# LayerXcom/zero-chain

Measured on NVIDIA H100. Metric: g1_msm_mops_2^20, higher is better.
Workload: dtype u32-limb Montgomery (Fq 12x32, Fr 8x32), integer

## Files before the change

zero_chain_b200/csrc/curve.cuh:

```cuda
#pragma once
#include "field.cuh"

struct Fq2 {
    Fq c0, c1;
    ZK_DEV static Fq2 zero() { Fq2 r; r.c0 = Fq::zero(); r.c1 = Fq::zero(); return r; }
    ZK_DEV static Fq2 one() { Fq2 r; r.c0 = Fq::one(); r.c1 = Fq::zero(); return r; }
    ZK_DEV bool is_zero() const { return c0.is_zero() && c1.is_zero(); }
    ZK_DEV bool operator==(const Fq2 &b) const { return c0 == b.c0 && c1 == b.c1; }
    ZK_DEV bool operator!=(const Fq2 &b) const { return !(*this == b); }
    ZK_DEV friend Fq2 operator+(const Fq2 &a, const Fq2 &b) { Fq2 r; r.c0 = a.c0 + b.c0; r.c1 = a.c1 + b.c1; return r; }
    ZK_DEV friend Fq2 operator-(const Fq2 &a, const Fq2 &b) { Fq2 r; r.c0 = a.c0 - b.c0; r.c1 = a.c1 - b.c1; return r; }
    ZK_DEV Fq2 dbl() const { Fq2 r; r.c0 = c0.dbl(); r.c1 = c1.dbl(); return r; }
    ZK_DEV Fq2 neg() const { Fq2 r; r.c0 = c0.neg(); r.c1 = c1.neg(); return r; }
    ZK_DEV Fq2 cneg(bool f) const { return f ? neg() : *this; }
    ZK_F2FN friend Fq2 operator*(const Fq2 &a, const Fq2 &b) {
        Fq aa = a.c0 * b.c0, bb = a.c1 * b.c1;
        Fq t = (a.c0 + a.c1) * (b.c0 + b.c1);
        Fq2 r; r.c1 = t - aa - bb; r.c0 = aa - bb; return r;
    }
    ZK_F2FN Fq2 sqr() const {
        Fq ab = c0 * c1;
        Fq2 r; r.c0 = (c0 + c1) * (c0 - c1); r.c1 = ab.dbl(); return r;
    }
    ZK_DEV Fq2 inverse() const {
        Fq n = (c0.sqr() + c1.sqr()).inverse();
        Fq2 r; r.c0 = c0 * n; r.c1 = (c1 * n).neg(); return r;
    }
};

template <class F>
struct Affine {
    F x, y;
    ZK_DEV bool is_inf() const { return x.is_zero() && y.is_zero(); }
    ZK_DEV static Affine inf() { Affine r; r.x = F::zero(); r.y = F::zero(); return r; }
};

template <class F>
struct XYZZ {
    F x, y, zz, zzz;
    ZK_DEV static XYZZ inf() { XYZZ r; r.x = F::zero(); r.y = F::zero(); r.zz = F::zero(); r.zzz = F::zero(); return r; }
    ZK_DEV bool is_inf() const { return zz.is_zero(); }
    ZK_DEV static XYZZ from_affine(const Affine<F> &p) {
        XYZZ r;
        if (p.is_inf()) return inf();
        r.x = p.x; r.y = p.y; r.zz = F::one(); r.zzz = F::one(); return r;
    }
    ZK_DEV XYZZ neg() const { XYZZ r = *this; r.y = y.neg(); return r; }

    ZK_PTFN static XYZZ dbl_affine(const Affine<F> &p) {
        if (p.is_inf()) return inf();
        F u = p.y.dbl(), v = u.sqr(), w = u * v, s = p.x * v;
        F xx = p.x.sqr(), m = xx.dbl() + xx;
        XYZZ r;
        r.x = m.sqr() - s.dbl();
        r.y = m * (s - r.x) - w * p.y;
        r.zz = v; r.zzz = w;
        return r;
    }
    ZK_PTFN XYZZ dbl() const {
        if (is_inf()) return *this;
        F u = y.dbl(), v = u.sqr(), w = u * v, s = x * v;
        F xx = x.sqr(), m = xx.dbl() + xx;
        XYZZ r;
        r.x = m.sqr() - s.dbl();
        r.y = m * (s - r.x) - w * y;
        r.zz = v * zz; r.zzz = w * zzz;
        return r;
    }
    ZK_PTFN void add_mixed(const Affine<F> &p) {
        if (p.is_inf()) return;
        if (is_inf()) { x = p.x; y = p.y; zz = F::one(); zzz = F::one(); return; }
        F u2 = p.x * zz, s2 = p.y * zzz;
        F pp_ = u2 - x, r = s2 - y;
        if (pp_.is_zero()) {
            if (r.is_zero()) *this = dbl_affine(p); else *this = inf();
            return;
        }
        F pp = pp_.sqr(), ppp = pp_ * pp, q = x * pp;
        F x3 = r.sqr() - ppp - q.dbl();
        y = r * (q - x3) - y * ppp;
        x = x3;
        zz = zz * pp; zzz = zzz * ppp;
    }
    ZK_PTFN void add(const XYZZ &o) {
        if (o.is_inf()) return;
        if (is_inf()) { *this = o; return; }
        F u1 = x * o.zz, u2 = o.x * zz, s1 = y * o.zzz, s2 = o.y * zzz;
        F pp_ = u2 - u1, r = s2 - s1;
        if (pp_.is_zero()) {
            if (r.is_zero()) *this = dbl(); else *this = inf();
            return;
        }
        F pp = pp_.sqr(), ppp = pp_ * pp, q = u1 * pp;
        F x3 = r.sqr() - ppp - q.dbl();
        y = r * (q - x3) - s1 * ppp;
        x = x3;
        zz = zz * o.zz * pp; zzz = zzz * o.zzz * ppp;
    }
    ZK_PTFN Affine<F> to_affine() const {
        if (is_inf()) return Affine<F>::inf();
        F zi = zzz.inverse();
        F zi2 = (zi * zz).sqr();
        Affine<F> r; r.x = x * zi2; r.y = y * zi; return r;
    }
};

template <class F>
ZK_PTFN XYZZ<F> scalar_mul(const XYZZ<F> &p, const uint32_t *k) {
    XYZZ<F> acc = XYZZ<F>::inf();
    bool started = false;
    for (int i = 255; i >= 0; i--) {
        if (started) acc = acc.dbl();
        if ((k[i >> 5] >> (i & 31)) & 1) { acc.add(p); started = true; }
    }
    return acc;
}

typedef Affine<Fq> G1Affine;
typedef Affine<Fq2> G2Affine;
typedef XYZZ<Fq> G1XYZZ;
typedef XYZZ<Fq2> G2XYZZ;
```

zero_chain_b200/csrc/curve_coop.cuh:

```cuda
#pragma once
#include "curve.cuh"

namespace zkcoop {

template <class F>
__device__ __forceinline__ F bcast(const F &v, int src) {
    F r;
    const uint32_t *s = reinterpret_cast<const uint32_t *>(&v);
    uint32_t *d = reinterpret_cast<uint32_t *>(&r);
#pragma unroll
    for (int k = 0; k < (int)(sizeof(F) / 4); k++) d[k] = __shfl_sync(0xffffffffu, s[k], src);
    return r;
}
template <class F>
__device__ __forceinline__ F pick(int lane, const F &c0, const F &c1, const F &c2, const F &c3) {
    F r;
    const uint32_t *p0 = reinterpret_cast<const uint32_t *>(&c0), *p1 = reinterpret_cast<const uint32_t *>(&c1);
    const uint32_t *p2 = reinterpret_cast<const uint32_t *>(&c2), *p3 = reinterpret_cast<const uint32_t *>(&c3);
    uint32_t *d = reinterpret_cast<uint32_t *>(&r);
#pragma unroll
    for (int k = 0; k < (int)(sizeof(F) / 4); k++) d[k] = lane == 1 ? p1[k] : (lane == 2 ? p2[k] : (lane == 3 ? p3[k] : p0[k]));
    return r;
}

template <class F>
__device__ __noinline__ void dbl(XYZZ<F> &P) {
    if (P.is_inf()) return;
    const int lane = threadIdx.x & 31;
    const F U = P.y.dbl();
    F a = pick(lane, U, P.x, U, U), p = a * a;
    const F V = bcast(p, 0), XX = bcast(p, 1);
    const F M = XX.dbl() + XX;
    a = pick(lane, U, P.x, M, U);
    F b = pick(lane, V, V, M, V);
    p = a * b;
    const F W = bcast(p, 0), S = bcast(p, 1), MM = bcast(p, 2);
    const F X3 = MM - S.dbl();
    a = pick(lane, M, W, V, W);
    b = pick(lane, S - X3, P.y, P.zz, P.zzz);
    p = a * b;
    const F t0 = bcast(p, 0), t1 = bcast(p, 1);
    P.zz = bcast(p, 2); P.zzz = bcast(p, 3);
    P.x = X3; P.y = t0 - t1;
}

template <class F>
__device__ __noinline__ void add(XYZZ<F> &P, const XYZZ<F> &Q) {
    if (Q.is_inf()) return;
    if (P.is_inf()) { P = Q; return; }
    const int lane = threadIdx.x & 31;
    F a = pick(lane, P.x, Q.x, P.y, Q.y), b = pick(lane, Q.zz, P.zz, Q.zzz, P.zzz), p = a * b;
    const F U1 = bcast(p, 0), U2 = bcast(p, 1), S1 = bcast(p, 2), S2 = bcast(p, 3);
    const F Pd = U2 - U1, R = S2 - S1;
    if (Pd.is_zero()) {
        if (R.is_zero()) dbl(P); else P = XYZZ<F>::inf();
        return;
    }
    a = pick(lane, Pd, R, P.zz, P.zzz); b = pick(lane, Pd, R, Q.zz, Q.zzz); p = a * b;
    const F PP = bcast(p, 0), RR = bcast(p, 1), ZZ12 = bcast(p, 2), ZZZ12 = bcast(p, 3);
    a = pick(lane, Pd, U1, ZZ12, Pd); p = a * PP;
    const F PPP = bcast(p, 0), Qv = bcast(p, 1);
    P.zz = bcast(p, 2);
    const F X3 = RR - PPP - Qv.dbl();
    a = pick(lane, R, S1, ZZZ12, R); b = pick(lane, Qv - X3, PPP, PPP, PPP); p = a * b;
    const F t0 = bcast(p, 0), t1 = bcast(p, 1);
    P.zzz = bcast(p, 2);
    P.x = X3; P.y = t0 - t1;
}

}
```

zero_chain_b200/csrc/engine.cu:

```cuda
#define ZK_SEMI_HOT 1
#include "internal.h"
#include "msm_driver.cuh"

using namespace zkmsm;

static thread_local char g_err[512] = "";
void zk_set_error(const char *fmt, ...) {
    va_list ap; va_start(ap, fmt); vsnprintf(g_err, sizeof(g_err), fmt, ap); va_end(ap);
    (void)cudaGetLastError();
}
extern "C" const char *zk_last_error(void) { return g_err; }
extern "C" const char *zk_version(void) { return "zkb200 0.1 (sm_90a)"; }
extern "C" int zk_device_count(void) {
    int n = 0;
    if (cudaGetDeviceCount(&n) != cudaSuccess) { cudaGetLastError(); return 0; }
    return n;
}
int zk_use_device(zk_ctx *ctx) { ZK_CUDA(cudaSetDevice(ctx->device)); return ZK_OK; }

extern "C" int zk_ctx_create(int device, void *stream, zk_ctx **out) {
    if (!out) { zk_set_error("zk_ctx_create: out is NULL"); return ZK_ERR_INVALID; }
    int n = zk_device_count();
    if (n == 0) { zk_set_error("no CUDA device: libzkb200 has no CPU fallback"); return ZK_ERR_CUDA; }
    if (device < 0 || device >= n) { zk_set_error("device %d out of range (%d devices)", device, n); return ZK_ERR_INVALID; }
// ... 244 lines not shown
    ctx->pending_bytes = 0;
    ZK_CUDA(cudaEventSynchronize(ctx->ev_tail));
    ZK_TRY(zk_check_err_flag(ctx));
    memcpy(out, ctx->h_pinned, per);
    return ZK_OK;
}
extern "C" size_t zk_partial_size(int group) { return group == 1 ? sizeof(G1XYZZ) : sizeof(G2XYZZ); }
extern "C" int zk_msm_partial_device(zk_ctx *ctx, const zk_bases *b, const void *d_scalars, size_t n, void *d_partial_out) {
    if (!d_partial_out) { zk_set_error("zk_msm_partial_device: out is NULL"); return ZK_ERR_INVALID; }
    ZK_TRY(zk_msm_run(ctx, b, d_scalars, n, 1));
    ZK_CUDA(cudaMemcpyAsync(d_partial_out, ctx->result.p, zk_partial_size(b->group), cudaMemcpyDeviceToDevice, ctx->stream));
    return zk_check_err_flag(ctx);
}
extern "C" int zk_points_fold(zk_ctx *ctx, int group, const void *d_partials, size_t count, uint8_t *out) {
    if (!ctx || !d_partials || !out || count == 0) { zk_set_error("zk_points_fold: bad argument"); return ZK_ERR_INVALID; }
    ZK_TRY(zk_use_device(ctx));
    ZK_TRY(ctx->result.reserve(4 * sizeof(G2XYZZ)));
    if (group == 1) k_fold_serial<Fq><<<1, 32, 0, ctx->stream>>>((const G1XYZZ *)d_partials, (int)count, ctx->result.as<G1XYZZ>());
    else k_fold_serial<Fq2><<<1, 32, 0, ctx->stream>>>((const G2XYZZ *)d_partials, (int)count, ctx->result.as<G2XYZZ>());
    ZK_CUDA(cudaGetLastError());
    return zk_encode_results(ctx, group, 1, 0, out);
}

template <class F>
__global__ void __launch_bounds__(128) k_scalar_mul_many(const Affine<F> *base, const uint32_t *scalars, size_t n, Affine<F> *out) {
    size_t i = (size_t)blockIdx.x * blockDim.x + threadIdx.x;
    if (i >= n) return;
    uint32_t k[8];
    for (int j = 0; j < 8; j++) k[j] = scalars[i * 8 + j];
    out[i] = scalar_mul(XYZZ<F>::from_affine(base[0]), k).to_affine();
}
extern "C" int zk_scalar_mul_many(zk_ctx *ctx, int group, const uint64_t *base, const uint64_t *scalars, size_t n, uint64_t *out) {
    if (!ctx || !base || !scalars || !out) { zk_set_error("zk_scalar_mul_many: NULL argument"); return ZK_ERR_INVALID; }
    if (group != 1 && group != 2) { zk_set_error("group must be 1 or 2"); return ZK_ERR_INVALID; }
    ZK_TRY(zk_use_device(ctx));
    size_t psz = group == 1 ? sizeof(G1Affine) : sizeof(G2Affine);
    ZK_TRY(ctx->stage_a.reserve(psz)); ZK_TRY(ctx->stage_b.reserve(n * 32)); ZK_TRY(ctx->stage_c.reserve(n * psz));
    ZK_CUDA(cudaMemcpyAsync(ctx->stage_a.p, base, psz, cudaMemcpyHostToDevice, ctx->stream));
    ZK_CUDA(cudaMemcpyAsync(ctx->stage_b.p, scalars, n * 32, cudaMemcpyHostToDevice, ctx->stream));
    unsigned blk = (unsigned)((n + 127) / 128);
    if (group == 1) k_scalar_mul_many<Fq><<<blk, 128, 0, ctx->stream>>>(ctx->stage_a.as<G1Affine>(), ctx->stage_b.as<uint32_t>(), n, ctx->stage_c.as<G1Affine>());
    else k_scalar_mul_many<Fq2><<<blk, 128, 0, ctx->stream>>>(ctx->stage_a.as<G2Affine>(), ctx->stage_b.as<uint32_t>(), n, ctx->stage_c.as<G2Affine>());
    ZK_CUDA(cudaGetLastError());
    ZK_CUDA(cudaMemcpyAsync(out, ctx->stage_c.p, n * psz, cudaMemcpyDeviceToHost, ctx->stream));
    ZK_CUDA(cudaStreamSynchronize(ctx->stream));
    return ZK_OK;
}

template <class T>
__global__ void k_field_op(int op, const T *a, const T *b, size_t n, T *out) {
    size_t i = (size_t)blockIdx.x * blockDim.x + threadIdx.x;
    if (i >= n) return;
    T x = a[i], y = b ? b[i] : x, r;
    switch (op) {
    case 0: r = x * y; break;
    case 1: r = x + y; break;
    case 2: r = x - y; break;
    case 3: r = x.sqr(); break;
    case 4: r = x.inverse(); break;
    case 5: r = T::canonical_lt_mod(x) ? T::from_canonical(x) : T::zero(); break;
    default: r = x.to_canonical(); break;
    }
    out[i] = r;
}
extern "C" int zk_field_op(zk_ctx *ctx, int field, int op, const uint64_t *a, const uint64_t *b, size_t n, uint64_t *out) {
    if (!ctx || !a || !out || op < 0 || op > 6 || (field != 0 && field != 1)) { zk_set_error("zk_field_op: bad argument"); return ZK_ERR_INVALID; }
    ZK_TRY(zk_use_device(ctx));
    size_t sz = field == 0 ? 48 : 32;
    ZK_TRY(ctx->stage_a.reserve(n * sz)); ZK_TRY(ctx->stage_b.reserve(n * sz)); ZK_TRY(ctx->stage_c.reserve(n * sz));
    ZK_CUDA(cudaMemcpyAsync(ctx->stage_a.p, a, n * sz, cudaMemcpyHostToDevice, ctx->stream));
    if (b) ZK_CUDA(cudaMemcpyAsync(ctx->stage_b.p, b, n * sz, cudaMemcpyHostToDevice, ctx->stream));
    unsigned blk = (unsigned)((n + 127) / 128);
    if (field == 0) k_field_op<Fq><<<blk, 128, 0, ctx->stream>>>(op, ctx->stage_a.as<Fq>(), b ? ctx->stage_b.as<Fq>() : nullptr, n, ctx->stage_c.as<Fq>());
    else k_field_op<Fr><<<blk, 128, 0, ctx->stream>>>(op, ctx->stage_a.as<Fr>(), b ? ctx->stage_b.as<Fr>() : nullptr, n, ctx->stage_c.as<Fr>());
    ZK_CUDA(cudaGetLastError());
    ZK_CUDA(cudaMemcpyAsync(out, ctx->stage_c.p, n * sz, cudaMemcpyDeviceToHost, ctx->stream));
    ZK_CUDA(cudaStreamSynchronize(ctx->stream));
    return ZK_OK;
}

extern "C" int zk_bench_modmul(zk_ctx *ctx, int field, int blocks, int threads, int iters, double *per_s, double *ms_out) {
    if (!ctx || !per_s) { zk_set_error("zk_bench_modmul: NULL argument"); return ZK_ERR_INVALID; }
#ifndef ZK_EXPERIMENTS
    if (field != 0 && field != 1) { zk_set_error("zk_bench_modmul: field must be 0 (Fq) or 1 (Fr)"); return ZK_ERR_INVALID; }
#endif
    ZK_TRY(zk_use_device(ctx));
    ZK_TRY(ctx->stage_a.reserve(64));
    cudaEvent_t e0, e1;
    ZK_CUDA(cudaEventCreate(&e0)); ZK_CUDA(cudaEventCreate(&e1));
    for (int rep = 0; rep < 2; rep++) {
        ZK_CUDA(cudaEventRecord(e0, ctx->stream));
        zk_launch_bench_modmul(field, blocks, threads, iters, ctx->stage_a.p, ctx->stream);
        ZK_CUDA(cudaEventRecord(e1, ctx->stream));
        ZK_CUDA(cudaEventSynchronize(e1));
    }
    float ms = 0;
    ZK_CUDA(cudaEventElapsedTime(&ms, e0, e1));
    cudaEventDestroy(e0); cudaEventDestroy(e1);
    *per_s = (double)blocks * threads * iters * 4.0 / (ms * 1e-3);
    if (ms_out) *ms_out = ms;
    return ZK_OK;
}

extern "C" int zk_ctx_profile(zk_ctx *ctx, int enable) {
    if (!ctx) { zk_set_error("zk_ctx_profile: NULL ctx"); return ZK_ERR_INVALID; }
    ZK_TRY(zk_use_device(ctx));
    ZK_CUDA(cudaStreamSynchronize(ctx->stream));
    for (cudaEvent_t ev : ctx->prof_events) cudaEventDestroy(ev);
    ctx->prof_events.clear();
    ctx->prof_on = enable != 0;
    for (zk_ctx *c : {ctx, ctx->aux, ctx->aux2, ctx->aux3})
        if (c) { ZK_CUDA(cudaStreamSynchronize(c->stream)); ZK_CUDA(cudaMemsetAsync(c->d_err + 10, 0, 8 * sizeof(int), c->stream)); ZK_CUDA(cudaStreamSynchronize(c->stream)); }
    return ZK_OK;
}
extern "C" int zk_ctx_profile_counts(zk_ctx *ctx, uint64_t *g1_additions, uint64_t *g2_additions, uint64_t *g1_xyzz, uint64_t *g2_xyzz) {
    if (!ctx || !g1_additions || !g2_additions || !g1_xyzz || !g2_xyzz) { zk_set_error("zk_ctx_profile_counts: NULL argument"); return ZK_ERR_INVALID; }
    ZK_TRY(zk_use_device(ctx));
    *g1_additions = 0; *g2_additions = 0; *g1_xyzz = 0; *g2_xyzz = 0;
    for (zk_ctx *c : {ctx, ctx->aux, ctx->aux2, ctx->aux3}) {
        if (!c) continue;
        unsigned long long v[4] = {0, 0, 0, 0};
        ZK_CUDA(cudaStreamSynchronize(c->stream));
        if (c->tail) ZK_CUDA(cudaStreamSynchronize(c->tail));
        ZK_CUDA(cudaMemcpy(v, c->d_err + 10, sizeof(v), cudaMemcpyDeviceToHost));
        *g1_additions += v[0]; *g2_additions += v[1]; *g1_xyzz += v[2]; *g2_xyzz += v[3];
    }
    return ZK_OK;
}
extern "C" int zk_ctx_profile_read(zk_ctx *ctx, double *total_ms, uint64_t *launches) {
    if (!ctx || !total_ms || !launches) { zk_set_error("zk_ctx_profile_read: NULL argument"); return ZK_ERR_INVALID; }
    ZK_TRY(zk_use_device(ctx));
    ZK_CUDA(cudaStreamSynchronize(ctx->stream));
    double tot = 0;
    for (size_t i = 0; i + 1 < ctx->prof_events.size(); i += 2) {
        float ms = 0;
        ZK_CUDA(cudaEventElapsedTime(&ms, ctx->prof_events[i], ctx->prof_events[i + 1]));
        tot += ms;
    }
    *total_ms = tot;
    *launches = ctx->prof_events.size() / 2;
    return ZK_OK;
}
```

zero_chain_b200/csrc/field.cuh:

```cuda
#pragma once
#include <stdint.h>

#ifdef ZK_HOST_EMUL
#define ZK_DEV inline
#define ZK_MULFN inline
#define ZK_PTFN inline
#define ZK_F2FN inline
#elif defined(ZK_HOT)
#define ZK_MULFN __device__ __forceinline__
#define ZK_PTFN __device__ __forceinline__
#elif defined(ZK_SEMI_HOT)
#define ZK_MULFN __device__ __forceinline__
#define ZK_PTFN __device__ __noinline__
#define ZK_F2FN __device__ __noinline__
#else
#define ZK_MULFN __device__ __noinline__
#define ZK_PTFN __device__ __noinline__
#endif
#ifdef ZK_HOST_EMUL
namespace zkprim {
static thread_local uint32_t cf = 0;
inline uint32_t add_cc(uint32_t a, uint32_t b) { uint64_t t = (uint64_t)a + b; cf = (uint32_t)(t >> 32); return (uint32_t)t; }
inline uint32_t addc_cc(uint32_t a, uint32_t b) { uint64_t t = (uint64_t)a + b + cf; cf = (uint32_t)(t >> 32); return (uint32_t)t; }
inline uint32_t addc(uint32_t a, uint32_t b) { return a + b + cf; }
// ... 80 lines not shown
        return m[i];
    }
};

template <class P>
struct alignas(16) Fp {
    static constexpr int N = P::N;
    uint32_t l[N];

    ZK_DEV static Fp zero() { Fp r; for (int i = 0; i < N; i++) r.l[i] = 0; return r; }
    ZK_DEV static Fp one() { Fp r; for (int i = 0; i < N; i++) r.l[i] = P::one(i); return r; }
    ZK_DEV bool is_zero() const { uint32_t o = 0; for (int i = 0; i < N; i++) o |= l[i]; return o == 0; }
    ZK_DEV bool operator==(const Fp &b) const { uint32_t o = 0; for (int i = 0; i < N; i++) o |= l[i] ^ b.l[i]; return o == 0; }
    ZK_DEV bool operator!=(const Fp &b) const { return !(*this == b); }

    ZK_DEV static Fp reduce_once(const Fp &t) {
        using namespace zkprim;
        Fp u;
        u.l[0] = sub_cc(t.l[0], P::mod(0));
#pragma unroll
        for (int i = 1; i < N; i++) u.l[i] = subc_cc(t.l[i], P::mod(i));
        uint32_t borrow = subc(0, 0);
        Fp r;
#pragma unroll
        for (int i = 0; i < N; i++) r.l[i] = borrow ? t.l[i] : u.l[i];
        return r;
    }
    ZK_DEV friend Fp operator+(const Fp &a, const Fp &b) {
        using namespace zkprim;
        Fp t;
        t.l[0] = add_cc(a.l[0], b.l[0]);
#pragma unroll
        for (int i = 1; i < N - 1; i++) t.l[i] = addc_cc(a.l[i], b.l[i]);
        t.l[N - 1] = addc(a.l[N - 1], b.l[N - 1]);
        return reduce_once(t);
    }
    ZK_DEV friend Fp operator-(const Fp &a, const Fp &b) {
        using namespace zkprim;
        Fp t;
        t.l[0] = sub_cc(a.l[0], b.l[0]);
#pragma unroll
        for (int i = 1; i < N; i++) t.l[i] = subc_cc(a.l[i], b.l[i]);
        uint32_t borrow = subc(0, 0);
        Fp r;
        r.l[0] = add_cc(t.l[0], borrow & P::mod(0));
#pragma unroll
        for (int i = 1; i < N - 1; i++) r.l[i] = addc_cc(t.l[i], borrow & P::mod(i));
        r.l[N - 1] = addc(t.l[N - 1], borrow & P::mod(N - 1));
        return r;
    }
    ZK_DEV Fp dbl() const { return *this + *this; }
    ZK_DEV Fp neg() const { return is_zero() ? *this : sub_raw_mod(*this); }
    ZK_DEV static Fp sub_raw_mod(const Fp &a) {
        using namespace zkprim;
        Fp r;
        r.l[0] = sub_cc(P::mod(0), a.l[0]);
#pragma unroll
        for (int i = 1; i < N - 1; i++) r.l[i] = subc_cc(P::mod(i), a.l[i]);
        r.l[N - 1] = subc(P::mod(N - 1), a.l[N - 1]);
        return r;
    }
    ZK_DEV Fp cneg(bool flag) const { return flag ? neg() : *this; }

    ZK_DEV static void row_first(uint32_t *even, uint32_t *odd, const uint32_t *a, uint32_t bi) {
        using namespace zkprim;
#pragma unroll
        for (int j = 0; j < N; j += 2) {
            even[j] = mul_lo(a[j], bi); even[j + 1] = mul_hi(a[j], bi);
            odd[j] = mul_lo(a[j + 1], bi); odd[j + 1] = mul_hi(a[j + 1], bi);
        }
    }
    template <class A>
    ZK_DEV static void cmad_even(uint32_t *acc, A a, uint32_t bi) {
        using namespace zkprim;
        acc[0] = mad_lo_cc(a(0), bi, acc[0]);
        acc[1] = madc_hi_cc(a(0), bi, acc[1]);
#pragma unroll
        for (int j = 2; j < N; j += 2) {
            acc[j] = madc_lo_cc(a(j), bi, acc[j]);
            acc[j + 1] = madc_hi_cc(a(j), bi, acc[j + 1]);
        }
    }
    ZK_DEV static void row(uint32_t *even, uint32_t *odd, const uint32_t *a, uint32_t bi) {
        using namespace zkprim;
        even[0] = add_cc(even[0], odd[1]);
#pragma unroll
        for (int j = 0; j < N - 2; j += 2) {
            odd[j] = madc_lo_cc(a[j + 1], bi, odd[j + 2]);
            odd[j + 1] = madc_hi_cc(a[j + 1], bi, odd[j + 3]);
        }
        odd[N - 2] = madc_lo_cc(a[N - 1], bi, 0);
        odd[N - 1] = madc_hi(a[N - 1], bi, 0);
        cmad_even(even, [&](int j) { return a[j]; }, bi);
        odd[N - 1] = addc(odd[N - 1], 0);
        reduce_row(even, odd);
    }
    ZK_DEV static void reduce_row(uint32_t *even, uint32_t *odd) {
        using namespace zkprim;
        uint32_t mi = even[0] * P::INV;
        odd[0] = mad_lo_cc(P::modc(1), mi, odd[0]);
        odd[1] = madc_hi_cc(P::modc(1), mi, odd[1]);
#pragma unroll
        for (int j = 2; j < N; j += 2) {
            odd[j] = madc_lo_cc(P::modc(j + 1), mi, odd[j]);
            odd[j + 1] = madc_hi_cc(P::modc(j + 1), mi, odd[j + 1]);
        }
        cmad_even(even, [](int j) { return P::modc(j); }, mi);
        odd[N - 1] = addc(odd[N - 1], 0);
    }
    ZK_MULFN friend Fp operator*(const Fp &a, const Fp &b) {
        using namespace zkprim;
        uint32_t even[N], odd[N];
        row_first(even, odd, a.l, b.l[0]);
        reduce_row(even, odd);
#pragma unroll
        for (int i = 1; i < N; i += 2) {
            row(odd, even, a.l, b.l[i]);
            if (i + 1 < N) row(even, odd, a.l, b.l[i + 1]);
        }
        Fp t;
        t.l[0] = add_cc(even[0], odd[1]);
#pragma unroll
        for (int k = 1; k < N - 1; k++) t.l[k] = addc_cc(even[k], odd[k + 1]);
        t.l[N - 1] = addc(even[N - 1], 0);
        return reduce_once(t);
    }
    ZK_DEV Fp sqr() const { return *this * *this; }

    ZK_DEV static Fp from_canonical(const Fp &x) { Fp r2; for (int i = 0; i < N; i++) r2.l[i] = P::r2(i); return x * r2; }
    ZK_DEV Fp to_canonical() const { Fp o = zero(); o.l[0] = 1; return *this * o; }
    ZK_DEV static bool canonical_lt_mod(const Fp &x) {
        using namespace zkprim;
        sub_cc(x.l[0], P::mod(0));
        uint32_t t;
#pragma unroll
        for (int i = 1; i < N; i++) t = subc_cc(x.l[i], P::mod(i));
        (void)t;
        return subc(0, 0) != 0;
    }
    ZK_PTFN Fp pow(const uint32_t *e, int nwords) const {
        Fp acc = one();
        bool started = false;
        for (int i = nwords * 32 - 1; i >= 0; i--) {
            if (started) acc = acc.sqr();
            if ((e[i >> 5] >> (i & 31)) & 1) { acc = acc * *this; started = true; }
        }
        return acc;
    }
    ZK_DEV static void raw_shr1(uint32_t *x) {
#pragma unroll
        for (int i = 0; i < N - 1; i++) x[i] = (x[i] >> 1) | (x[i + 1] << 31);
        x[N - 1] >>= 1;
    }
    ZK_DEV static void raw_half_mod(uint32_t *x) {
        using namespace zkprim;
        uint32_t m = (x[0] & 1u) ? 0xffffffffu : 0u;
        x[0] = add_cc(x[0], m & P::mod(0));
#pragma unroll
        for (int i = 1; i < N - 1; i++) x[i] = addc_cc(x[i], m & P::mod(i));
        x[N - 1] = addc(x[N - 1], m & P::mod(N - 1));
        raw_shr1(x);
    }
    ZK_DEV static bool raw_is_one(const uint32_t *x) {
        uint32_t o = x[0] ^ 1u;
#pragma unroll
        for (int i = 1; i < N; i++) o |= x[i];
        return o == 0;
    }
    ZK_DEV static bool raw_lt(const uint32_t *x, const uint32_t *y) {
        using namespace zkprim;
        sub_cc(x[0], y[0]);
        uint32_t t = 0;
#pragma unroll
        for (int i = 1; i < N; i++) t = subc_cc(x[i], y[i]);
        (void)t;
        return subc(0, 0) != 0;
    }
    ZK_DEV static void raw_sub(uint32_t *x, const uint32_t *y) {
        using namespace zkprim;
        x[0] = sub_cc(x[0], y[0]);
#pragma unroll
        for (int i = 1; i < N - 1; i++) x[i] = subc_cc(x[i], y[i]);
        x[N - 1] = subc(x[N - 1], y[N - 1]);
    }
    ZK_PTFN Fp inverse() const {
        if (is_zero()) return *this;
        uint32_t u[N], v[N];
        Fp b, c = zero();
#pragma unroll
        for (int i = 0; i < N; i++) { u[i] = l[i]; v[i] = P::mod(i); b.l[i] = P::r2(i); }
        while (!raw_is_one(u) && !raw_is_one(v)) {
            while (!(u[0] & 1u)) { raw_shr1(u); raw_half_mod(b.l); }
            while (!(v[0] & 1u)) { raw_shr1(v); raw_half_mod(c.l); }
            if (raw_lt(v, u)) { raw_sub(u, v); b = b - c; }
            else { raw_sub(v, u); c = c - b; }
        }
        return raw_is_one(u) ? b : c;
    }
    ZK_PTFN Fp inverse_fermat() const {
        uint32_t e[N];
        uint32_t borrow = 2;
        for (int i = 0; i < N; i++) { uint32_t v = P::mod(i); e[i] = v - borrow; borrow = (v < borrow) ? 1u : 0u; }
        return pow(e, N);
    }
};

typedef Fp<FqParams> Fq;
typedef Fp<FrParams> Fr;
```

zero_chain_b200/csrc/msm_affine_core.cuh:

```cuda
#pragma once
#include "curve.cuh"

namespace zkmsm {

enum { PAIR_ADD = 0, PAIR_DBL = 1, PAIR_COPY0 = 2, PAIR_COPY1 = 3, PAIR_INF = 4 };

template <class F>
struct PairIO {
    const Affine<F> *pts;
    const uint32_t *sorted;
    ZK_DEV Affine<F> load(uint32_t i) const {
        Affine<F> p;
        if (sorted) {
            uint32_t code = sorted[i];
            p = pts[code & 0x7fffffffu];
            p.y = p.y.cneg(code >> 31);
        } else p = pts[i];
        return p;
    }
};

template <class F>
ZK_DEV int pair_classify(const Affine<F> &p0, const Affine<F> &p1, bool has1, F &den) {
    den = F::one();
    if (!has1 || p1.is_inf()) return PAIR_COPY0;
    if (p0.is_inf()) return PAIR_COPY1;
    if (p0.x == p1.x) {
        if (p0.y == p1.y) {
            den = p0.y.dbl();
            if (!den.is_zero()) return PAIR_DBL;
            den = F::one();
            return PAIR_INF;
        }
        return PAIR_INF;
    }
    den = p1.x - p0.x;
    return PAIR_ADD;
}
template <class F>
ZK_DEV Affine<F> pair_finish(int mode, const Affine<F> &p0, const Affine<F> &p1, const F &dinv) {
    if (mode == PAIR_COPY0) return p0;
    if (mode == PAIR_COPY1) return p1;
    if (mode == PAIR_INF) return Affine<F>::inf();
    F lam;
    if (mode == PAIR_DBL) { F xx = p0.x.sqr(); lam = (xx.dbl() + xx) * dinv; }
    else lam = (p1.y - p0.y) * dinv;
    Affine<F> r;
    r.x = lam.sqr() - p0.x - p1.x;
    r.y = lam * (p0.x - r.x) - p0.y;
    return r;
}

}
```

zero_chain_b200/csrc/msm_batchaff.cuh:

```cuda
#pragma once
#include <cuda_runtime.h>
#include <stdint.h>
#include "curve.cuh"
#include "msm_affine_core.cuh"
#include "msm_warp_scan.cuh"

namespace zkmsm {

constexpr int BA_T = 128;
constexpr int BA_K = 32;
constexpr int BA_MINB = 4;
constexpr int BA_MAX_LEVELS = 8;
constexpr int BA_INV_T = 512;
constexpr uint32_t BA_NONE = 0xffffffffu;

static __global__ void k_half_sizes(const uint32_t *__restrict__ off_in, uint32_t *__restrict__ sizes_out, uint32_t n_buckets) {
    uint32_t b = blockIdx.x * blockDim.x + threadIdx.x;
    if (b < n_buckets) sizes_out[b] = (off_in[b + 1] - off_in[b] + 1) >> 1;
}

template <class F>
__device__ __forceinline__ void ba_store_f(F *dst, const F &v) {
    const uint4 *s = reinterpret_cast<const uint4 *>(&v);
    uint4 *d = reinterpret_cast<uint4 *>(dst);
// ... 95 lines not shown
    const uint32_t total = off_out[n_buckets];
    const uint32_t n = ((total + BA_T * K - 1) / (BA_T * K)) * (BA_T / 32);
    const int t = threadIdx.x;
    const uint32_t per = (n + BA_INV_T - 1) / BA_INV_T, c0 = t * per, c1 = c0 + per < n ? c0 + per : n;
    F run = F::one();
    for (uint32_t i = c0; i < c1; i++) { ba_store_f(scratch + i, run); run = run * ba_load_f(totals + i); }
    node[BA_INV_T + t] = run;
    for (int s = BA_INV_T / 2; s >= 1; s >>= 1) {
        __syncthreads();
        if (t < s) node[s + t] = node[2 * (s + t)] * node[2 * (s + t) + 1];
    }
    __syncthreads();
    if (t == 0) node[1] = node[1].inverse();
    for (int s = 1; s < BA_INV_T; s <<= 1) {
        __syncthreads();
        if (t < s) {
            F inv = node[s + t], l = node[2 * (s + t)], r = node[2 * (s + t) + 1];
            node[2 * (s + t)] = inv * r;
            node[2 * (s + t) + 1] = inv * l;
        }
    }
    __syncthreads();
    F inv = node[BA_INV_T + t];
    for (uint32_t i = c1; i-- > c0;) {
        F v = ba_load_f(totals + i);
        ba_store_f(inv_out + i, inv * ba_load_f(scratch + i));
        inv = inv * v;
    }
}

template <class F, bool FIRST, int MINB>
__global__ void __launch_bounds__(BA_T, MINB) k_ba_backward(const Affine<F> *__restrict__ in_pts, const uint32_t *__restrict__ off_out, uint32_t n_buckets, int K,
                                                             const F *__restrict__ prefix, const uint2 *__restrict__ srcs, const F *__restrict__ block_inv,
                                                             Affine<F> *__restrict__ out_pts) {
    constexpr int PV = (int)(sizeof(Affine<F>) / 16), FV = (int)(sizeof(F) / 16);
    extern __shared__ unsigned char ba_smem[];
    uint4 *stage = reinterpret_cast<uint4 *>(ba_smem);
    const uint32_t total = off_out[n_buckets];
    const uint32_t n_blocks = (total + BA_T * K - 1) / (BA_T * K);
    if (blockIdx.x >= n_blocks) return;
    const int t = threadIdx.x;
    const size_t T_total = (size_t)gridDim.x * BA_T, tid = (size_t)blockIdx.x * BA_T + t;
    const uint32_t o0 = (uint32_t)tid * K;
    if (o0 >= total) return;
    F inv = ba_load_f(block_inv + (tid >> 5)) * ba_load_f(prefix + (size_t)K * T_total + tid);
    const uint32_t o1 = o0 + K < total ? o0 + K : total;
    uint4 *slot = stage + t;
    auto prefetch = [&](uint32_t o) {
        uint2 src = srcs[o];
        const uint4 *a = reinterpret_cast<const uint4 *>(ba_addr<F, FIRST>(in_pts, src.x));
        const uint4 *b = reinterpret_cast<const uint4 *>(ba_addr<F, FIRST>(in_pts, src.y == BA_NONE ? src.x : src.y));
        const uint4 *c = reinterpret_cast<const uint4 *>(prefix + (size_t)(o - o0) * T_total + tid);
#pragma unroll
        for (int v = 0; v < PV; v++) {
            asm volatile("cp.async.cg.shared.global [%0], [%1], 16;" ::"r"((uint32_t)__cvta_generic_to_shared(slot + v * BA_T)), "l"(a + v) : "memory");
            asm volatile("cp.async.cg.shared.global [%0], [%1], 16;" ::"r"((uint32_t)__cvta_generic_to_shared(slot + (PV + v) * BA_T)), "l"(b + v) : "memory");
        }
#pragma unroll
        for (int v = 0; v < FV; v++)
            asm volatile("cp.async.cg.shared.global [%0], [%1], 16;" ::"r"((uint32_t)__cvta_generic_to_shared(slot + (2 * PV + v) * BA_T)), "l"(c + v) : "memory");
        asm volatile("cp.async.commit_group;" ::: "memory");
        return src;
    };
    uint2 src = prefetch(o1 - 1);
    for (uint32_t o = o1; o-- > o0;) {
        asm volatile("cp.async.wait_group 0;" ::: "memory");
        Affine<F> p0, p1;
        F pre;
        {
            uint4 *d0 = reinterpret_cast<uint4 *>(&p0), *d1 = reinterpret_cast<uint4 *>(&p1), *d2 = reinterpret_cast<uint4 *>(&pre);
#pragma unroll
            for (int v = 0; v < PV; v++) { d0[v] = slot[v * BA_T]; d1[v] = slot[(PV + v) * BA_T]; }
#pragma unroll
            for (int v = 0; v < FV; v++) d2[v] = slot[(2 * PV + v) * BA_T];
        }
        const uint2 cur = src;
        if (o > o0) src = prefetch(o - 1);
        const bool has1 = cur.y != BA_NONE;
        if (FIRST) { p0.y = p0.y.cneg(cur.x >> 31); if (has1) p1.y = p1.y.cneg(cur.y >> 31); }
        if (!has1) p1 = Affine<F>::inf();
        F den;
        const int mode = pair_classify(p0, p1, has1, den);
        F dinv = F::one();
        if (mode <= PAIR_DBL) { dinv = inv * pre; inv = inv * den; }
        Affine<F> r = pair_finish(mode, p0, p1, dinv);
        uint4 *dst = reinterpret_cast<uint4 *>(out_pts + o);
        const uint4 *rs = reinterpret_cast<const uint4 *>(&r);
#pragma unroll
        for (int v = 0; v < PV; v++) dst[v] = rs[v];
    }
}

template <class F> constexpr size_t ba_smem_forward() { return 0; }
template <class F> constexpr size_t ba_smem_backward() { return (size_t)BA_T * (2 * sizeof(Affine<F>) + sizeof(F)); }
template <class F> constexpr size_t ba_smem_invert() { return 2 * BA_INV_T * sizeof(F); }

}
```

zero_chain_b200/csrc/msm_hot.cu:

```cuda
#define ZK_HOT 1
#include "msm_driver.cuh"
#ifdef ZK_EXPERIMENTS
#include "field_wide.cuh"
#endif

using namespace zkmsm;

int zk_msm_run_g1(zk_ctx *ctx, const zk_bases *b, const uint32_t *d_scalars, size_t n, size_t batch) { return msm_run_t<Fq>(ctx, b, d_scalars, n, batch); }
int zk_build_tables_g1(zk_ctx *ctx, zk_bases *b) { return build_tables_t<Fq>(ctx, b); }
int zk_encode_results_g1(zk_ctx *ctx, size_t count, int compressed, uint8_t *d_out) { return encode_results_t<Fq>(ctx, count, compressed, d_out); }

template <class T>
__global__ void k_bench_modmul(int iters, T *sink) {
    T a[4], b = T::one();
    for (int k = 0; k < 4; k++) { a[k] = T::one(); a[k].l[0] += threadIdx.x + k + 1; }
    b.l[1] ^= blockIdx.x + 7;
    a[0] = T::reduce_once(a[0]); b = T::reduce_once(b);
    for (int i = 0; i < iters; i++) {
#pragma unroll
        for (int k = 0; k < 4; k++) a[k] = a[k] * b;
    }
    T r = a[0] + a[1] + a[2] + a[3];
    if (r.l[0] == 0x12345678u && r.l[1] == 0x9abcdef0u) sink[0] = r;
}
#ifdef ZK_EXPERIMENTS
template <int MODE>
__global__ void k_bench_wide(int iters, Fq *sink) {
    Fq a[4], b = Fq::one();
    for (int k = 0; k < 4; k++) { a[k] = Fq::one(); a[k].l[0] += threadIdx.x + k + 1; }
    b.l[1] ^= blockIdx.x + 7;
    a[0] = Fq::reduce_once(a[0]); b = Fq::reduce_once(b);
    for (int i = 0; i < iters; i++) {
#pragma unroll
        for (int k = 0; k < 4; k++) {
            if (MODE == 0) a[k] = a[k] * b;
            else if (MODE == 1) a[k] = zkwide::mul_sep(a[k], b);
            else if (MODE == 2) a[k] = a[k] * a[k];
            else if (MODE == 3) a[k] = zkwide::sqr_sep(a[k]);
            else if (MODE == 4) a[k] = a[k] * b - b * a[(k + 1) & 3];
            else a[k] = zkwide::mul_sub_mul(a[k], b, b, a[(k + 1) & 3]);
        }
    }
    Fq r = a[0] + a[1] + a[2] + a[3];
    if (r.l[0] == 0x12345678u && r.l[1] == 0x9abcdef0u) sink[0] = r;
}
#endif
void zk_launch_bench_modmul(int field, int blocks, int threads, int iters, void *sink, cudaStream_t st) {
    if (field == 0) k_bench_modmul<Fq><<<blocks, threads, 0, st>>>(iters, (Fq *)sink);
    else if (field == 1) k_bench_modmul<Fr><<<blocks, threads, 0, st>>>(iters, (Fr *)sink);
#ifdef ZK_EXPERIMENTS
    else if (field == 10) k_bench_wide<0><<<blocks, threads, 0, st>>>(iters, (Fq *)sink);
    else if (field == 11) k_bench_wide<1><<<blocks, threads, 0, st>>>(iters, (Fq *)sink);
    else if (field == 12) k_bench_wide<2><<<blocks, threads, 0, st>>>(iters, (Fq *)sink);
    else if (field == 13) k_bench_wide<3><<<blocks, threads, 0, st>>>(iters, (Fq *)sink);
    else if (field == 14) k_bench_wide<4><<<blocks, threads, 0, st>>>(iters, (Fq *)sink);
    else k_bench_wide<5><<<blocks, threads, 0, st>>>(iters, (Fq *)sink);
#endif
}
```

zero_chain_b200/groth16.py:

```python
from __future__ import annotations

import ctypes as C
import secrets

import numpy as np

from . import _lib
from ._lib import ZkError, check

R_MODULUS = 0x73eda753299d7d483339d80809a1d80553bda402fffe5bfeffffffff00000001


class SynthesisError(Exception):
    NAMES = {-3: "AssignmentMissing", -4: "PolynomialDegreeTooLarge", -5: "UnexpectedIdentity", -6: "IoError",
             -7: "IoError(GroupDecodingError)", -8: "IoError(NotInField)", -9: "MalformedVerifyingKey"}

    def __init__(self, code, msg):
        super().__init__("%s: %s" % (self.NAMES.get(code, "Error(%d)" % code), msg))
        self.code = code


def _ck(code):
    if code == 0:
        return
# ... 353 lines not shown


def create_random_proof(prover: ProvingAssignment, params: Parameters, rng=None) -> bytes:
    draw = (lambda: secrets.randbelow(R_MODULUS)) if rng is None else (lambda: rng.randrange(R_MODULUS))
    return create_proof(prover, params, draw(), draw())


def create_proof_batch(provers, params: Parameters, rs, ss) -> bytes:
    p0 = provers[0]
    batch = len(provers)
    cat = lambda name: np.ascontiguousarray(np.concatenate([getattr(p, name) for p in provers], axis=0))
    a, b, c, inp, aux = (cat(k) for k in ("a", "b", "c", "input_assignment", "aux_assignment"))
    rr = np.stack([_fr_limbs(x) for x in rs]); sv = np.stack([_fr_limbs(x) for x in ss])
    out = np.zeros(192 * batch, np.uint8)
    _ck(_lib.lib().zk_groth16_prove_batch(params.ctx._h, params._h, batch, _p(a), _p(b), _p(c), p0.a.shape[0],
                                          _p(inp), p0.input_assignment.shape[0], _p(aux), p0.aux_assignment.shape[0],
                                          _p(p0.a_aux_density), _p(p0.b_input_density), _p(p0.b_aux_density),
                                          _p(rr), _p(sv), _p(out)))
    return out.tobytes()


class ConstraintSystem:

    def __init__(self, ctx: Context, n_inputs: int, n_aux: int, rows_a, rows_b, rows_c):
        self.ctx, self.n_inputs, self.n_aux = ctx, n_inputs, n_aux
        n_c = len(rows_a)
        assert len(rows_b) == n_c and len(rows_c) == n_c
        arrs = []
        for rows in (rows_a, rows_b, rows_c):
            rp = np.zeros(n_c + 1, np.uint32)
            rp[1:] = np.cumsum([len(r) for r in rows])
            col = np.array([v for r in rows for v, _ in r] or [0], np.uint32)
            cf = np.zeros((max(1, int(rp[-1])), 4), np.uint64)
            k = 0
            for r in rows:
                for _, c in r:
                    for j in range(4):
                        cf[k, j] = (c >> (64 * j)) & 0xFFFFFFFFFFFFFFFF
                    k += 1
            arrs += [rp, col, cf]
        self._h = C.c_void_p()
        _ck(_lib.lib().zk_r1cs_load(ctx._h, n_c, n_inputs, n_aux, *[_p(a) for a in arrs], C.byref(self._h)))

    def free(self):
        if self._h:
            _lib.lib().zk_r1cs_free(self._h)
            self._h = C.c_void_p()

    def __del__(self):
        try:
            self.free()
        except Exception:
            pass


def create_proof_from_witness_batch(cs: ConstraintSystem, params: Parameters, batch: int, inputs, aux, r, s) -> bytes:
    inputs, aux = _u64(inputs, (batch, cs.n_inputs, 4)), _u64(aux, (batch, cs.n_aux, 4))
    r, s = _u64(r, (batch, 4)), _u64(s, (batch, 4))
    out = np.zeros(192 * batch, np.uint8)
    _ck(_lib.lib().zk_groth16_prove_witness_batch(params.ctx._h, params._h, cs._h, batch, _p(inputs), _p(aux), _p(r), _p(s), _p(out)))
    return out.tobytes()


def create_proof_batch_raw(params: Parameters, batch: int, a, b, c, inputs, aux, a_aux_density, b_input_density, b_aux_density, r, s) -> bytes:
    a, b, c, inputs, aux = (_u64(x, (batch, -1, 4)) for x in (a, b, c, inputs, aux))
    r, s = _u64(r, (batch, 4)), _u64(s, (batch, 4))
    d1, d2, d3 = (np.ascontiguousarray(x, np.uint8) for x in (a_aux_density, b_input_density, b_aux_density))
    out = np.zeros(192 * batch, np.uint8)
    _ck(_lib.lib().zk_groth16_prove_batch(params.ctx._h, params._h, batch, _p(a), _p(b), _p(c), a.shape[1],
                                          _p(inputs), inputs.shape[1], _p(aux), aux.shape[1], _p(d1), _p(d2), _p(d3), _p(r), _p(s), _p(out)))
    return out.tobytes()


def scalar_mul_many(ctx: Context, group: int, base_limbs, scalars):
    s = _u64(scalars, (-1, 4))
    w = 12 if group == 1 else 24
    base = _u64(base_limbs, (w,))
    out = np.zeros((s.shape[0], w), np.uint64)
    _ck(_lib.lib().zk_scalar_mul_many(ctx._h, group, _p(base), _p(s), s.shape[0], _p(out)))
    return out


FIELD_FQ, FIELD_FR = 0, 1
OP_MUL, OP_ADD, OP_SUB, OP_SQR, OP_INV, OP_FROM_REPR, OP_INTO_REPR = range(7)


def field_op(ctx: Context, field: int, op: int, a, b=None):
    nl = 6 if field == 0 else 4
    a = _u64(a, (-1, nl))
    bb = None if b is None else _u64(b, (-1, nl))
    out = np.zeros_like(a)
    _ck(_lib.lib().zk_field_op(ctx._h, field, op, _p(a), _p(bb) if bb is not None else None, a.shape[0], _p(out)))
    return out


def bench_modmul(ctx: Context, field: int, blocks: int, threads: int, iters: int):
    per_s, ms = C.c_double(), C.c_double()
    _ck(_lib.lib().zk_bench_modmul(ctx._h, field, blocks, threads, iters, C.byref(per_s), C.byref(ms)))
    return per_s.value, ms.value


G1_GENERATOR = np.array([0x5cb38790fd530c16, 0x7817fc679976fff5, 0x154f95c7143ba1c1, 0xf0ae6acdf3d0e747, 0xedce6ecc21dbf440, 0x120177419e0bfb75,
                         0xbaac93d50ce72271, 0x8c22631a7918fd8e, 0xdd595f13570725ce, 0x51ac582950405194, 0x0e1c8c3fad0059c0, 0x0bbc3efc5008a26a], np.uint64)
G2_GENERATOR = np.array([0xf5f28fa202940a10, 0xb3f5fb2687b4961a, 0xa1a893b53e2ae580, 0x9894999d1a3caee9, 0x6f67b7631863366b, 0x058191924350bcd7,
                         0xa5a9c0759e23f606, 0xaaa0c59dbccd60c3, 0x3bb17e18e2867806, 0x1b1ab6cc8541b367, 0xc2b6ed0ef2158547, 0x11922a097360edf3,
                         0x4c730af860494c4a, 0x597cfa1f5e369c5a, 0xe7e6856caa0a635a, 0xbbefb5e96e0d495f, 0x07d3a975f0ef25a2, 0x0083fd8e7e80dae5,
                         0xadc0fc92df64b05d, 0x18aa270a2b1461dc, 0x86adac6a3be4eba0, 0x79495c4ec93da33a, 0xe7175850a43ccaed, 0x0b2bc2a163de1bf2], np.uint64)
```

Before: 125.3.

## Add dedicated Montgomery squaring, fused mul-sub-mul, and lazy reduction in curve ops

Adds a dedicated squaring routine that computes the cross products once and doubles them, followed by a separate Montgomery reduction. Adds a fused a*b - c*d that interleaves two products into one reduction, and lazy (unreduced) multiplies for Fq. These are used in XYZZ doubling and addition, in batch-affine pair finishing and in the inverse chain, to cut modular multiply work and final conditional subtractions. The cost is tighter bounds on intermediate values (guarded by static_asserts on the modulus size), more complex carry chains that could raise register pressure, and a new squaring benchmark mode.

Result: faster. 126.7 (median of 6 runs) (+1.1%).

```diff
diff --git a/zero_chain_b200/csrc/curve.cuh b/zero_chain_b200/csrc/curve.cuh
--- a/zero_chain_b200/csrc/curve.cuh
+++ b/zero_chain_b200/csrc/curve.cuh
@@ -28,6 +28,13 @@
     }
 };
 
+template <class F> ZK_DEV F mul_lz(const F &a, const F &b) { return a * b; }
+template <class F> ZK_DEV F sqr_lz(const F &a) { return a.sqr(); }
+ZK_DEV Fq mul_lz(const Fq &a, const Fq &b) { return Fq::mul_lazy(a, b); }
+ZK_DEV Fq sqr_lz(const Fq &a) { return a.sqr_lazy(); }
+template <class F> ZK_DEV F mul_sub_mul(const F &a, const F &b, const F &c, const F &d) { return a * b - c * d; }
+ZK_DEV Fq mul_sub_mul(const Fq &a, const Fq &b, const Fq &c, const Fq &d) { return Fq::mul_sub_mul(a, b, c, d); }
+
 template <class F>
 struct Affine {
     F x, y;
@@ -53,17 +60,17 @@
         F xx = p.x.sqr(), m = xx.dbl() + xx;
         XYZZ r;
         r.x = m.sqr() - s.dbl();
-        r.y = m * (s - r.x) - w * p.y;
+        r.y = mul_sub_mul(m, s - r.x, w, p.y);
         r.zz = v; r.zzz = w;
         return r;
     }
     ZK_PTFN XYZZ dbl() const {
         if (is_inf()) return *this;
-        F u = y.dbl(), v = u.sqr(), w = u * v, s = x * v;
+        F u = y.dbl(), v = sqr_lz(u), w = mul_lz(u, v), s = x * v;
         F xx = x.sqr(), m = xx.dbl() + xx;
         XYZZ r;
         r.x = m.sqr() - s.dbl();
-        r.y = m * (s - r.x) - w * y;
+        r.y = mul_sub_mul(m, s - r.x, w, y);
         r.zz = v * zz; r.zzz = w * zzz;
         return r;
     }
@@ -91,11 +98,11 @@
             if (r.is_zero()) *this = dbl(); else *this = inf();
             return;
         }
-        F pp = pp_.sqr(), ppp = pp_ * pp, q = u1 * pp;
+        F pp = sqr_lz(pp_), ppp = pp_ * pp, q = u1 * pp;
         F x3 = r.sqr() - ppp - q.dbl();
-        y = r * (q - x3) - s1 * ppp;
+        y = mul_sub_mul(r, q - x3, s1, ppp);
         x = x3;
-        zz = zz * o.zz * pp; zzz = zzz * o.zzz * ppp;
+        zz = mul_lz(zz, o.zz) * pp; zzz = mul_lz(zzz, o.zzz) * ppp;
     }
     ZK_PTFN Affine<F> to_affine() const {
         if (is_inf()) return Affine<F>::inf();
diff --git a/zero_chain_b200/csrc/curve_coop.cuh b/zero_chain_b200/csrc/curve_coop.cuh
--- a/zero_chain_b200/csrc/curve_coop.cuh
+++ b/zero_chain_b200/csrc/curve_coop.cuh
@@ -28,7 +28,7 @@
     if (P.is_inf()) return;
     const int lane = threadIdx.x & 31;
     const F U = P.y.dbl();
-    F a = pick(lane, U, P.x, U, U), p = a * a;
+    F a = pick(lane, U, P.x, U, U), p = a.sqr();
     const F V = bcast(p, 0), XX = bcast(p, 1);
     const F M = XX.dbl() + XX;
     a = pick(lane, U, P.x, M, U);
diff --git a/zero_chain_b200/csrc/engine.cu b/zero_chain_b200/csrc/engine.cu
--- a/zero_chain_b200/csrc/engine.cu
+++ b/zero_chain_b200/csrc/engine.cu
@@ -350,7 +350,7 @@
 extern "C" int zk_bench_modmul(zk_ctx *ctx, int field, int blocks, int threads, int iters, double *per_s, double *ms_out) {
     if (!ctx || !per_s) { zk_set_error("zk_bench_modmul: NULL argument"); return ZK_ERR_INVALID; }
 #ifndef ZK_EXPERIMENTS
-    if (field != 0 && field != 1) { zk_set_error("zk_bench_modmul: field must be 0 (Fq) or 1 (Fr)"); return ZK_ERR_INVALID; }
+    if (field < 0 || field > 2) { zk_set_error("zk_bench_modmul: field must be 0 (Fq), 1 (Fr) or 2 (Fq squaring)"); return ZK_ERR_INVALID; }
 #endif
     ZK_TRY(zk_use_device(ctx));
     ZK_TRY(ctx->stage_a.reserve(64));
diff --git a/zero_chain_b200/csrc/field.cuh b/zero_chain_b200/csrc/field.cuh
--- a/zero_chain_b200/csrc/field.cuh
+++ b/zero_chain_b200/csrc/field.cuh
@@ -186,6 +186,10 @@
         }
     }
     ZK_DEV static void row(uint32_t *even, uint32_t *odd, const uint32_t *a, uint32_t bi) {
+        row_shift(even, odd, a, bi);
+        reduce_row(even, odd);
+    }
+    ZK_DEV static void row_shift(uint32_t *even, uint32_t *odd, const uint32_t *a, uint32_t bi) {
         using namespace zkprim;
         even[0] = add_cc(even[0], odd[1]);
 #pragma unroll
@@ -197,22 +201,33 @@
         odd[N - 1] = madc_hi(a[N - 1], bi, 0);
         cmad_even(even, [&](int j) { return a[j]; }, bi);
         odd[N - 1] = addc(odd[N - 1], 0);
-        reduce_row(even, odd);
+    }
+    template <class A>
+    ZK_DEV static void mad_row(uint32_t *even, uint32_t *odd, A a, uint32_t bi) {
+        using namespace zkprim;
+        odd[0] = mad_lo_cc(a(1), bi, odd[0]);
+        odd[1] = madc_hi_cc(a(1), bi, odd[1]);
+#pragma unroll
+        for (int j = 2; j < N; j += 2) {
+            odd[j] = madc_lo_cc(a(j + 1), bi, odd[j]);
+            odd[j + 1] = madc_hi_cc(a(j + 1), bi, odd[j + 1]);
+        }
+        cmad_even(even, a, bi);
+        odd[N - 1] = addc(odd[N - 1], 0);
     }
     ZK_DEV static void reduce_row(uint32_t *even, uint32_t *odd) {
-        using namespace zkprim;
-        uint32_t mi = even[0] * P::INV;
-        odd[0] = mad_lo_cc(P::modc(1), mi, odd[0]);
-        odd[1] = madc_hi_cc(P::modc(1), mi, odd[1]);
-#pragma unroll
-        for (int j = 2; j < N; j += 2) {
-            odd[j] = madc_lo_cc(P::modc(j + 1), mi, odd[j]);
-            odd[j + 1] = madc_hi_cc(P::modc(j + 1), mi, odd[j + 1]);
-        }
-        cmad_even(even, [](int j) { return P::modc(j); }, mi);
-        odd[N - 1] = addc(odd[N - 1], 0);
-    }
-    ZK_MULFN friend Fp operator*(const Fp &a, const Fp &b) {
+        mad_row(even, odd, [](int j) { return P::modc(j); }, even[0] * P::INV);
+    }
+    ZK_DEV static Fp finish_rows(const uint32_t *even, const uint32_t *odd) {
+        using namespace zkprim;
+        Fp t;
+        t.l[0] = add_cc(even[0], odd[1]);
+#pragma unroll
+        for (int k = 1; k < N - 1; k++) t.l[k] = addc_cc(even[k], odd[k + 1]);
+        t.l[N - 1] = addc(even[N - 1], 0);
+        return t;
+    }
+    ZK_DEV static Fp mul_unreduced(const Fp &a, const Fp &b) {
         using namespace zkprim;
         uint32_t even[N], odd[N];
         row_first(even, odd, a.l, b.l[0]);
@@ -222,14 +237,131 @@
             row(odd, even, a.l, b.l[i]);
             if (i + 1 < N) row(even, odd, a.l, b.l[i + 1]);
         }
-        Fp t;
-        t.l[0] = add_cc(even[0], odd[1]);
-#pragma unroll
-        for (int k = 1; k < N - 1; k++) t.l[k] = addc_cc(even[k], odd[k + 1]);
-        t.l[N - 1] = addc(even[N - 1], 0);
-        return reduce_once(t);
-    }
-    ZK_DEV Fp sqr() const { return *this * *this; }
+        return finish_rows(even, odd);
+    }
+    ZK_DEV static Fp mul_add_mul_unreduced(const Fp &a, const Fp &b, const Fp &c, const Fp &d) {
+        static_assert(P::mod(N - 1) < 0x20000000u, "a fused sum of products needs p < R/8");
+        uint32_t even[N], odd[N];
+        row_first(even, odd, a.l, b.l[0]);
+        mad_row(even, odd, [&](int j) { return c.l[j]; }, d.l[0]);
+        reduce_row(even, odd);
+#pragma unroll
+        for (int i = 1; i < N; i += 2) {
+            row_shift(odd, even, a.l, b.l[i]);
+            mad_row(odd, even, [&](int j) { return c.l[j]; }, d.l[i]);
+            reduce_row(odd, even);
+            if (i + 1 < N) {
+                row_shift(even, odd, a.l, b.l[i + 1]);
+                mad_row(even, odd, [&](int j) { return c.l[j]; }, d.l[i + 1]);
+                reduce_row(even, odd);
+            }
+        }
+        return finish_rows(even, odd);
+    }
+
+    ZK_DEV static int cross_row(uint32_t *acc, int top, const uint32_t *a, int i, int j0) {
+        using namespace zkprim;
+        if (j0 >= N) return top;
+        int jl = j0;
+        while (jl + 2 < N) jl += 2;
+        if (i + j0 >= top) {
+#pragma unroll
+            for (int j = j0; j < N; j += 2) { acc[i + j] = mul_lo(a[i], a[j]); acc[i + j + 1] = mul_hi(a[i], a[j]); }
+            return i + jl + 2;
+        }
+#pragma unroll
+        for (int j = j0; j < N; j += 2) {
+            const int p = i + j;
+            const uint32_t lo = p < top ? acc[p] : 0u, hi = p + 1 < top ? acc[p + 1] : 0u;
+            acc[p] = j == j0 ? mad_lo_cc(a[i], a[j], lo) : madc_lo_cc(a[i], a[j], lo);
+            if (j == jl && p + 1 >= top) { acc[p + 1] = madc_hi(a[i], a[j], 0u); return p + 2; }
+            acc[p + 1] = madc_hi_cc(a[i], a[j], hi);
+        }
+#pragma unroll
+        for (int k = i + jl + 2; k < top; k++) acc[k] = addc_cc(acc[k], 0u);
+        acc[top] = addc(0u, 0u);
+        return top + 1;
+    }
+    ZK_DEV static void sqr_wide(uint32_t *t, const uint32_t *a) {
+        using namespace zkprim;
+        uint32_t o[2 * N], e[2 * N];
+        int to = 0, te = 0;
+#pragma unroll
+        for (int i = 0; i < N - 1; i++) {
+            to = cross_row(o, to, a, i, i + 1);
+            te = cross_row(e, te, a, i, i + 2);
+        }
+#pragma unroll
+        for (int k = to; k < 2 * N; k++) o[k] = 0;
+#pragma unroll
+        for (int k = te; k < 2 * N; k++) e[k] = 0;
+        o[2] = add_cc(o[2], e[2]);
+#pragma unroll
+        for (int k = 3; k < 2 * N - 1; k++) o[k] = addc_cc(o[k], e[k]);
+        o[2 * N - 1] = addc(o[2 * N - 1], e[2 * N - 1]);
+#pragma unroll
+        for (int k = 2 * N - 1; k > 1; k--) t[k] = (o[k] << 1) | (o[k - 1] >> 31);
+        t[1] = o[1] << 1;
+        t[0] = mul_lo(a[0], a[0]);
+        t[1] = mad_hi_cc(a[0], a[0], t[1]);
+#pragma unroll
+        for (int i = 1; i < N - 1; i++) {
+            t[2 * i] = madc_lo_cc(a[i], a[i], t[2 * i]);
+            t[2 * i + 1] = madc_hi_cc(a[i], a[i], t[2 * i + 1]);
+        }
+        t[2 * N - 2] = madc_lo_cc(a[N - 1], a[N - 1], t[2 * N - 2]);
+        t[2 * N - 1] = madc_hi(a[N - 1], a[N - 1], t[2 * N - 1]);
+    }
+    ZK_DEV static void redc_row(uint32_t *even, uint32_t *odd, uint32_t hi) {
+        using namespace zkprim;
+        const uint32_t mi = (even[0] + odd[1]) * P::INV;
+        even[0] = add_cc(even[0], odd[1]);
+#pragma unroll
+        for (int j = 0; j < N - 2; j += 2) {
+            odd[j] = madc_lo_cc(P::modc(j + 1), mi, odd[j + 2]);
+            odd[j + 1] = madc_hi_cc(P::modc(j + 1), mi, odd[j + 3]);
+        }
+        odd[N - 2] = madc_lo_cc(P::modc(N - 1), mi, hi);
+        odd[N - 1] = madc_hi(P::modc(N - 1), mi, 0u);
+        cmad_even(even, [](int j) { return P::modc(j); }, mi);
+        odd[N - 1] = addc(odd[N - 1], 0u);
+    }
+    ZK_DEV static Fp sqr_unreduced(const Fp &a) {
+        using namespace zkprim;
+        uint32_t t[2 * N], odd[N];
+        sqr_wide(t, a.l);
+        uint32_t *even = t;
+        const uint32_t m0 = even[0] * P::INV;
+#pragma unroll
+        for (int j = 0; j < N; j += 2) { odd[j] = mul_lo(P::modc(j + 1), m0); odd[j + 1] = mul_hi(P::modc(j + 1), m0); }
+        cmad_even(even, [](int j) { return P::modc(j); }, m0);
+        odd[N - 1] = addc(odd[N - 1], 0u);
+#pragma unroll
+        for (int i = 1; i < N; i += 2) {
+            redc_row(odd, even, t[N + i - 1]);
+            if (i + 1 < N) redc_row(even, odd, t[N + i]);
+        }
+        Fp r;
+        r.l[0] = add_cc(even[0], odd[1]);
+#pragma unroll
+        for (int k = 1; k < N - 1; k++) r.l[k] = addc_cc(even[k], odd[k + 1]);
+        r.l[N - 1] = addc(even[N - 1], t[2 * N - 1]);
+        return r;
+    }
+
+    ZK_MULFN friend Fp operator*(const Fp &a, const Fp &b) { return reduce_once(mul_unreduced(a, b)); }
+    ZK_MULFN Fp sqr() const { return reduce_once(sqr_unreduced(*this)); }
+    ZK_MULFN static Fp mul_sub_mul(const Fp &a, const Fp &b, const Fp &c, const Fp &d) {
+        return reduce_once(mul_add_mul_unreduced(a, b, c, d.neg()));
+    }
+    ZK_MULFN static Fp mul_lazy(const Fp &a, const Fp &b) {
+        static_assert(P::mod(N - 1) < 0x40000000u, "lazy reduction needs p < R/4");
+        return mul_unreduced(a, b);
+    }
+    ZK_MULFN Fp sqr_lazy() const {
+        static_assert(P::mod(N - 1) < 0x40000000u, "lazy reduction needs p < R/4");
+        return sqr_unreduced(*this);
+    }
 
     ZK_DEV static Fp from_canonical(const Fp &x) { Fp r2; for (int i = 0; i < N; i++) r2.l[i] = P::r2(i); return x * r2; }
     ZK_DEV Fp to_canonical() const { Fp o = zero(); o.l[0] = 1; return *this * o; }
diff --git a/zero_chain_b200/csrc/msm_affine_core.cuh b/zero_chain_b200/csrc/msm_affine_core.cuh
--- a/zero_chain_b200/csrc/msm_affine_core.cuh
+++ b/zero_chain_b200/csrc/msm_affine_core.cuh
@@ -43,8 +43,8 @@
     if (mode == PAIR_COPY1) return p1;
     if (mode == PAIR_INF) return Affine<F>::inf();
     F lam;
-    if (mode == PAIR_DBL) { F xx = p0.x.sqr(); lam = (xx.dbl() + xx) * dinv; }
-    else lam = (p1.y - p0.y) * dinv;
+    if (mode == PAIR_DBL) { F xx = p0.x.sqr(); lam = mul_lz(xx.dbl() + xx, dinv); }
+    else lam = mul_lz(p1.y - p0.y, dinv);
     Affine<F> r;
     r.x = lam.sqr() - p0.x - p1.x;
     r.y = lam * (p0.x - r.x) - p0.y;
diff --git a/zero_chain_b200/csrc/msm_batchaff.cuh b/zero_chain_b200/csrc/msm_batchaff.cuh
--- a/zero_chain_b200/csrc/msm_batchaff.cuh
+++ b/zero_chain_b200/csrc/msm_batchaff.cuh
@@ -201,7 +201,7 @@
         F den;
         const int mode = pair_classify(p0, p1, has1, den);
         F dinv = F::one();
-        if (mode <= PAIR_DBL) { dinv = inv * pre; inv = inv * den; }
+        if (mode <= PAIR_DBL) { dinv = mul_lz(inv, pre); inv = mul_lz(inv, den); }
         Affine<F> r = pair_finish(mode, p0, p1, dinv);
         uint4 *dst = reinterpret_cast<uint4 *>(out_pts + o);
         const uint4 *rs = reinterpret_cast<const uint4 *>(&r);
diff --git a/zero_chain_b200/csrc/msm_hot.cu b/zero_chain_b200/csrc/msm_hot.cu
--- a/zero_chain_b200/csrc/msm_hot.cu
+++ b/zero_chain_b200/csrc/msm_hot.cu
@@ -10,7 +10,7 @@
 int zk_build_tables_g1(zk_ctx *ctx, zk_bases *b) { return build_tables_t<Fq>(ctx, b); }
 int zk_encode_results_g1(zk_ctx *ctx, size_t count, int compressed, uint8_t *d_out) { return encode_results_t<Fq>(ctx, count, compressed, d_out); }
 
-template <class T>
+template <class T, bool SQR = false>
 __global__ void k_bench_modmul(int iters, T *sink) {
     T a[4], b = T::one();
     for (int k = 0; k < 4; k++) { a[k] = T::one(); a[k].l[0] += threadIdx.x + k + 1; }
@@ -18,7 +18,7 @@
     a[0] = T::reduce_once(a[0]); b = T::reduce_once(b);
     for (int i = 0; i < iters; i++) {
 #pragma unroll
-        for (int k = 0; k < 4; k++) a[k] = a[k] * b;
+        for (int k = 0; k < 4; k++) a[k] = SQR ? a[k].sqr() : a[k] * b;
     }
     T r = a[0] + a[1] + a[2] + a[3];
     if (r.l[0] == 0x12345678u && r.l[1] == 0x9abcdef0u) sink[0] = r;
@@ -48,6 +48,7 @@
 void zk_launch_bench_modmul(int field, int blocks, int threads, int iters, void *sink, cudaStream_t st) {
     if (field == 0) k_bench_modmul<Fq><<<blocks, threads, 0, st>>>(iters, (Fq *)sink);
     else if (field == 1) k_bench_modmul<Fr><<<blocks, threads, 0, st>>>(iters, (Fr *)sink);
+    else if (field == 2) k_bench_modmul<Fq, true><<<blocks, threads, 0, st>>>(iters, (Fq *)sink);
 #ifdef ZK_EXPERIMENTS
     else if (field == 10) k_bench_wide<0><<<blocks, threads, 0, st>>>(iters, (Fq *)sink);
     else if (field == 11) k_bench_wide<1><<<blocks, threads, 0, st>>>(iters, (Fq *)sink);
diff --git a/zero_chain_b200/groth16.py b/zero_chain_b200/groth16.py
--- a/zero_chain_b200/groth16.py
+++ b/zero_chain_b200/groth16.py
@@ -459,6 +459,7 @@
 
 
 FIELD_FQ, FIELD_FR = 0, 1
+BENCH_FQ_SQR = 2
 OP_MUL, OP_ADD, OP_SUB, OP_SQR, OP_INV, OP_FROM_REPR, OP_INTO_REPR = range(7)
 
 
```
